# FFTAI/Wiki-GRx-Gym

Hardware: AMD Instinct MI355X
Metric: env-steps/sec GR1T1 rough-terrain @4096 envs (higher is better)
Workload: dtype f32

## Files before the change

### include/grx_ppo.h

```cpp
#ifndef GRX_PPO_H
#define GRX_PPO_H
#ifdef __cplusplus
extern "C" {
#endif

int grx_ppo_loss_partials_size(int batch);

int grx_ppo_loss(int batch, int num_actions, const float* mu, const float* std, const float* value,
                 const float* actions, const float* old_logp, const float* old_mu, const float* old_sigma,
                 const float* advantages, const float* returns, const float* target_values,
                 float clip_param, float value_loss_coef, float entropy_coef, int use_clipped_value_loss,
                 float* out, float* d_mu, float* d_std, float* d_value, float* partials, void* stream);

int grx_ppo_colsum_partials_size(int rows, int cols);
int grx_ppo_colsum(int rows, int cols, const float* x, float* out, float* partials, void* stream);

int grx_ppo_elu_backward_colsum(int rows, int cols, const float* dy, const float* y, float* dz, float* out, float* partials, void* stream);

int grx_ppo_store_transition(int N, int num_obs, int num_pri, int num_actions,
                             const float* obs, const float* pri, const float* actions, const float* mu, const float* sigma,
                             const float* values, const float* logp, const float* rewards, const unsigned char* dones,
                             const unsigned char* time_outs, float gamma,
                             float* st_obs, float* st_pri, float* st_actions, float* st_mu, float* st_sigma, float* st_values,
                             float* st_logp, float* st_rewards, unsigned char* st_dones,
                             float* cur_rew, float* cur_len, float* done_rew, float* done_len, void* stream);

#define GRX_PPO_TAIL_MAX 24
typedef struct grx_ppo_tail_tensors {
    int n, pad;
    float* param[GRX_PPO_TAIL_MAX]; const float* grad[GRX_PPO_TAIL_MAX]; float* exp_avg[GRX_PPO_TAIL_MAX]; float* exp_avg_sq[GRX_PPO_TAIL_MAX];
    float* step[GRX_PPO_TAIL_MAX];
    long long numel[GRX_PPO_TAIL_MAX];
} grx_ppo_tail_tensors;
typedef struct grx_ppo_tail_args {
    const float* loss;
    const float* bad_flag;
    const float* kl;
    float* lr;
    const float *value_loss, *surrogate_loss;
    float* sums;
    float* partials;
    int adaptive, pad;
    float desired_kl, lr_min, lr_max, max_grad_norm;
    double beta1, beta2, eps;
} grx_ppo_tail_args;
int grx_ppo_step_tail_blocks(const grx_ppo_tail_tensors* t);
int grx_ppo_step_tail(const grx_ppo_tail_tensors* t, const grx_ppo_tail_args* a, void* stream);

#define GRX_PPO_GATHER_MAX 12
int grx_ppo_gather_rows(int n_tensors, const float* const* src, float* const* dst, const int* widths, const long long* idx, int mb, void* stream);

int grx_mlp_layer(int M, int K, int N, const float* X, const float* W, const float* bias, float* Y, int elu, void* stream);

int grx_mlp_layer_bf16(int M, int K, int N, const float* X, const float* W, const float* bias, float* Y, int elu, void* stream);
int grx_mlp_input_grad_bf16(int M, int N, int K, const float* dZ, const float* W, float* dX, void* stream);
int grx_mlp_weight_grad_bf16_partials_size(int M, int N, int K);
int grx_mlp_weight_grad_bf16(int M, int N, int K, const float* dZ, const float* X, float* dW, float* partials, void* stream);

int grx_mlp_policy_head(int M, int K, int A, const float* X, const float* W, const float* bias, const float* std,
                        const float* eps, float* actions, float* logp, float* mu, float* sigma, void* stream);

int grx_obs_norm_partials_size(int rows, int cols);
int grx_obs_norm_moments(int rows, int cols, const float* x, float* partials, void* stream);
int grx_obs_norm_merge(int n_partials, int cols, int stride, const float* partials, long long* count, float* mean, float* var, float* std,
                       void* stream);
int grx_obs_norm_combine(int n_partials, int cols, const float* partials, float* out, void* stream);
int grx_obs_norm_apply(int rows, int cols, const float* x, const float* mean, const float* std, float eps, float* y, void* stream);
int grx_obs_norm_step(int rows, int cols, const float* x, float* partials, long long* count, float* mean, float* var, float* std, float eps,
                      float* y, void* stream);

int grx_obs_history_push(int N, int D, int H, const float* obs, const unsigned char* dones, int fill_all, const float* src, float* dst,
                         void* stream);

int grx_distill_loss_partials_size(int batch, int A);
int grx_distill_loss(int batch, int A, const float* student_mu, const float* teacher_mu, int huber, float* out, float* d_mu, float* partials,
                     void* stream);
int grx_distill_store(int N, int D, int A, const float* obs, const float* labels, const float* rewards, const unsigned char* dones,
                      float* st_obs, float* st_labels, unsigned char* st_dones,
                      float* cur_rew, float* cur_len, float* done_rew, float* done_len, void* stream);

int grx_lstm_cell(int M, int D, int H, const float* x, const float* h_prev, const float* c_prev, const unsigned char* reset,
                  const float* W_ih, const float* W_hh, const float* b_ih, const float* b_hh, float* h, float* c, float* acts, void* stream);
int grx_lstm_cell_preact(int M, int D, int H, const float* x, const float* h_prev, const unsigned char* reset, const float* W_ih,
                         const float* W_hh, const float* b_ih, const float* b_hh, float* G, void* stream);
int grx_lstm_cell_backward(int M, int H, const float* dh, const float* dc_in, const float* acts, const float* c_prev,
                           const unsigned char* reset, float* dG, float* dc_prev, void* stream);

#define GRX_SYM_MAX_WIDTH 2048
int grx_sym_gather_rows(int n_tensors, const float* const* src, float* const* dst, const int* widths, const int* modes,
                        const int* const* perm, const float* const* scale, const float* const* offset, const long long* idx, int mb,
                        void* stream);

int grx_rnd_reward_partials_size(int N);
int grx_rnd_reward(int N, int E, const float* pred, const float* targ, float gamma, float weight, float eps, float* ret, long long* count,
                   float* mean, float* var, float* std, float* rewards, float* intrinsic, float* raw, float* partials, void* stream);

#ifdef __cplusplus
}
#endif

#include "grx_ppo_noise.h"
#include "grx_ppo_smooth.h"
#include "grx_ppo_est.h"
#endif
```

### wiki-grx-gym_amd/rl/fused_loss.py

```python
import ctypes as C
import os

import torch

_LIB = None


def load_ppo_library():
    global _LIB
    if _LIB is None:
        path = os.environ.get("GRX_PPO_LIB") or os.path.join(os.path.dirname(os.path.dirname(os.path.abspath(__file__))), "csrc", "libgrx_ppo.so")
        if not os.path.exists(path):
            raise RuntimeError(f"{path} is missing: build it with `python -c 'import __graft_entry__ as g; g.build()'` "
                               "(there is no silent fallback for CUDA tensors; set GRX_PPO_FUSED_LOSS=0 to use the torch expression)")
        lib = C.CDLL(path)
        fp = C.c_void_p
        lib.grx_ppo_loss.restype = C.c_int
        lib.grx_ppo_loss.argtypes = [C.c_int, C.c_int] + [fp] * 10 + [C.c_float, C.c_float, C.c_float, C.c_int] + [fp] * 5 + [C.c_void_p]
        lib.grx_ppo_loss_partials_size.restype = C.c_int
        lib.grx_ppo_loss_partials_size.argtypes = [C.c_int]
        lib.grx_ppo_colsum.restype = C.c_int
        lib.grx_ppo_colsum.argtypes = [C.c_int, C.c_int, fp, fp, fp, C.c_void_p]
        lib.grx_ppo_colsum_partials_size.restype = C.c_int
        lib.grx_ppo_colsum_partials_size.argtypes = [C.c_int, C.c_int]
        lib.grx_ppo_store_transition.restype = C.c_int
        lib.grx_ppo_store_transition.argtypes = [C.c_int] * 4 + [fp] * 10 + [C.c_float] + [fp] * 13 + [C.c_void_p]
        lib.grx_ppo_elu_backward_colsum.restype = C.c_int
        lib.grx_ppo_elu_backward_colsum.argtypes = [C.c_int, C.c_int, fp, fp, fp, fp, fp, C.c_void_p]
        lib.grx_ppo_gather_rows.restype = C.c_int
        lib.grx_ppo_gather_rows.argtypes = [C.c_int, C.POINTER(C.c_void_p), C.POINTER(C.c_void_p), C.POINTER(C.c_int), fp, C.c_int, C.c_void_p]
        lib.grx_mlp_layer.restype = C.c_int
        lib.grx_mlp_layer.argtypes = [C.c_int] * 3 + [fp] * 4 + [C.c_int, C.c_void_p]
        lib.grx_mlp_layer_bf16.restype = C.c_int
        lib.grx_mlp_layer_bf16.argtypes = [C.c_int] * 3 + [fp] * 4 + [C.c_int, C.c_void_p]
        lib.grx_mlp_input_grad_bf16.restype = C.c_int
        lib.grx_mlp_input_grad_bf16.argtypes = [C.c_int] * 3 + [fp] * 3 + [C.c_void_p]
        lib.grx_mlp_weight_grad_bf16_partials_size.restype = C.c_int
        lib.grx_mlp_weight_grad_bf16_partials_size.argtypes = [C.c_int] * 3
        lib.grx_mlp_weight_grad_bf16.restype = C.c_int
        lib.grx_mlp_weight_grad_bf16.argtypes = [C.c_int] * 3 + [fp] * 4 + [C.c_void_p]
        lib.grx_mlp_policy_head.restype = C.c_int
        lib.grx_mlp_policy_head.argtypes = [C.c_int] * 3 + [fp] * 9 + [C.c_void_p]
        lib.grx_ppo_step_tail.restype = C.c_int
        lib.grx_ppo_step_tail.argtypes = [C.c_void_p, C.c_void_p, C.c_void_p]
        lib.grx_ppo_step_tail_blocks.restype = C.c_int
        lib.grx_ppo_step_tail_blocks.argtypes = [C.c_void_p]
        lib.grx_obs_norm_partials_size.restype = C.c_int
        lib.grx_obs_norm_partials_size.argtypes = [C.c_int, C.c_int]
        lib.grx_obs_norm_moments.restype = C.c_int
        lib.grx_obs_norm_moments.argtypes = [C.c_int, C.c_int, fp, fp, C.c_void_p]
        lib.grx_obs_norm_merge.restype = C.c_int
        lib.grx_obs_norm_merge.argtypes = [C.c_int, C.c_int, C.c_int] + [fp] * 5 + [C.c_void_p]
        lib.grx_obs_norm_combine.restype = C.c_int
        lib.grx_obs_norm_combine.argtypes = [C.c_int, C.c_int, fp, fp, C.c_void_p]
        lib.grx_obs_norm_apply.restype = C.c_int
        lib.grx_obs_norm_apply.argtypes = [C.c_int, C.c_int, fp, fp, fp, C.c_float, fp, C.c_void_p]
        lib.grx_obs_norm_step.restype = C.c_int
        lib.grx_obs_norm_step.argtypes = [C.c_int, C.c_int] + [fp] * 6 + [C.c_float, fp, C.c_void_p]
        lib.grx_obs_history_push.restype = C.c_int
        lib.grx_obs_history_push.argtypes = [C.c_int] * 3 + [fp, fp, C.c_int, fp, fp, C.c_void_p]
        lib.grx_distill_loss_partials_size.restype = C.c_int
        lib.grx_distill_loss_partials_size.argtypes = [C.c_int, C.c_int]
        lib.grx_distill_loss.restype = C.c_int
        lib.grx_distill_loss.argtypes = [C.c_int, C.c_int, fp, fp, C.c_int, fp, fp, fp, C.c_void_p]
        lib.grx_distill_store.restype = C.c_int
        lib.grx_distill_store.argtypes = [C.c_int] * 3 + [fp] * 11 + [C.c_void_p]
        pp = C.POINTER(C.c_void_p)
        lib.grx_sym_gather_rows.restype = C.c_int
        lib.grx_sym_gather_rows.argtypes = [C.c_int, pp, pp, C.POINTER(C.c_int), C.POINTER(C.c_int), pp, pp, pp, fp, C.c_int, C.c_void_p]
        lib.grx_rnd_reward_partials_size.restype = C.c_int
        lib.grx_rnd_reward_partials_size.argtypes = [C.c_int]
        lib.grx_rnd_reward.restype = C.c_int
        lib.grx_rnd_reward.argtypes = [C.c_int, C.c_int, fp, fp, C.c_float, C.c_float, C.c_float] + [fp] * 9 + [C.c_void_p]
        lib.grx_ppo_loss_sd_partials_size.restype = C.c_int
        lib.grx_ppo_loss_sd_partials_size.argtypes = [C.c_int]
        lib.grx_ppo_loss_sd.restype = C.c_int
        lib.grx_ppo_loss_sd.argtypes = [C.c_int, C.c_int, fp, C.c_int] + [fp] * 8 + [C.c_float, C.c_float, C.c_float, C.c_int] + [fp] * 4 + [C.c_void_p]
        lib.grx_mlp_policy_head_sd.restype = C.c_int
        lib.grx_mlp_policy_head_sd.argtypes = [C.c_int] * 3 + [fp] * 3 + [C.c_int] + [fp] * 5 + [C.c_void_p]
        lib.grx_smooth_gather_rows.restype = C.c_int
        lib.grx_smooth_gather_rows.argtypes = ([C.c_int, pp, pp, C.POINTER(C.c_int), fp, C.c_int, C.c_int, C.c_int, fp, C.c_int, C.c_int, fp,
                                                C.c_float, fp, C.c_void_p])
        lib.grx_smooth_loss_partials_size.restype = C.c_int
        lib.grx_smooth_loss_partials_size.argtypes = [C.c_int, C.c_int]
        lib.grx_smooth_loss.restype = C.c_int
        lib.grx_smooth_loss.argtypes = [C.c_int, C.c_int, fp, C.c_int, C.c_int, fp, C.c_float, C.c_float, fp, fp, fp, C.c_void_p]
        lib.grx_est_forward.restype = C.c_int
        lib.grx_est_forward.argtypes = [fp, C.c_int, C.c_int, fp, C.c_int, fp, C.POINTER(C.c_int), fp, fp, C.c_void_p]
        _LIB = lib
    return _LIB


TAIL_MAX = 24


class _TailTensors(C.Structure):
    _fields_ = [("n", C.c_int), ("pad", C.c_int), ("param", C.c_void_p * TAIL_MAX), ("grad", C.c_void_p * TAIL_MAX),
                ("exp_avg", C.c_void_p * TAIL_MAX), ("exp_avg_sq", C.c_void_p * TAIL_MAX), ("step", C.c_void_p * TAIL_MAX),
                ("numel", C.c_longlong * TAIL_MAX)]


class _TailArgs(C.Structure):
    _fields_ = [("loss", C.c_void_p), ("bad_flag", C.c_void_p), ("kl", C.c_void_p), ("lr", C.c_void_p), ("value_loss", C.c_void_p),
                ("surrogate_loss", C.c_void_p), ("sums", C.c_void_p), ("partials", C.c_void_p), ("adaptive", C.c_int), ("pad", C.c_int),
                ("desired_kl", C.c_float), ("lr_min", C.c_float), ("lr_max", C.c_float), ("max_grad_norm", C.c_float),
                ("beta1", C.c_double), ("beta2", C.c_double), ("eps", C.c_double)]


class StepTail:

    @staticmethod
    def supported(optimizer, params):
        g = optimizer.param_groups
        return (len(g) == 1 and len(params) <= TAIL_MAX and not g[0].get("amsgrad") and not g[0].get("maximize") and g[0].get("weight_decay", 0) == 0
                and all(p.is_cuda and p.dtype == torch.float32 and p.is_contiguous() for p in params))

    def __init__(self, optimizer, params, lr_t):
        self.lib = load_ppo_library()
        self.opt, self.params, self.lr_t = optimizer, list(params), lr_t
        self.t, self.a = _TailTensors(), _TailArgs()
        self.key, self.partials = None, None

    def _state(self, p):
        st = self.opt.state[p]
        if "exp_avg" not in st:
            st["step"] = torch.zeros((), dtype=torch.float32, device=p.device)
            st["exp_avg"] = torch.zeros_like(p, memory_format=torch.preserve_format)
            st["exp_avg_sq"] = torch.zeros_like(p, memory_format=torch.preserve_format)
        return st

    def __call__(self, loss, kl, value_loss, surrogate_loss, sums, adaptive, desired_kl, lr_min, lr_max, max_grad_norm, bad_flag=None):
        t, a = self.t, self.a
        sts = [self._state(p) for p in self.params]
        key = tuple(x.data_ptr() for p, st in zip(self.params, sts) for x in (p, st["exp_avg"], st["exp_avg_sq"], st["step"]))
        if key != self.key:
            t.n = len(self.params)
            for i, (p, st) in enumerate(zip(self.params, sts)):
                if not (st["step"].is_cuda and st["step"].dtype == torch.float32 and st["exp_avg"].is_contiguous() and st["exp_avg_sq"].is_contiguous()):
                    raise RuntimeError("StepTail: the optimizer state is not torch's fused / capturable layout")
                t.param[i], t.exp_avg[i], t.exp_avg_sq[i], t.step[i], t.numel[i] = p.data_ptr(), st["exp_avg"].data_ptr(), st["exp_avg_sq"].data_ptr(), st["step"].data_ptr(), p.numel()
            nb = self.lib.grx_ppo_step_tail_blocks(C.byref(t))
            if nb < 1:
                raise RuntimeError("grx_ppo_step_tail_blocks failed")
            self.partials = torch.empty(nb, device=self.params[0].device, dtype=torch.float32)
            self.key = key
        for i, p in enumerate(self.params):
            g = p.grad
            if g is None or not g.is_contiguous() or g.dtype != torch.float32:
                raise RuntimeError("StepTail: every parameter needs a contiguous fp32 .grad")
            t.grad[i] = g.data_ptr()
        g0 = self.opt.param_groups[0]
        a.loss, a.kl, a.lr = loss.data_ptr(), kl.data_ptr(), self.lr_t.data_ptr()
        a.bad_flag = bad_flag.data_ptr() if bad_flag is not None else None
        a.value_loss, a.surrogate_loss = value_loss.data_ptr(), surrogate_loss.data_ptr()
        a.sums = sums.data_ptr() if sums is not None else None
        a.partials = self.partials.data_ptr()
        a.adaptive = int(bool(adaptive))
        a.desired_kl, a.lr_min, a.lr_max, a.max_grad_norm = float(desired_kl or 0.0), float(lr_min), float(lr_max), float(max_grad_norm)
        a.beta1, a.beta2, a.eps = float(g0["betas"][0]), float(g0["betas"][1]), float(g0["eps"])
        dev = self.params[0].device
        with torch.cuda.device(dev):
            rc = self.lib.grx_ppo_step_tail(C.byref(t), C.byref(a), C.c_void_p(torch.cuda.current_stream(dev).cuda_stream))
        if rc != 0:
            raise RuntimeError(f"grx_ppo_step_tail failed ({rc})")


def _f32c(x):
    return x if (x.dtype == torch.float32 and x.is_contiguous()) else x.contiguous().float()


class FusedPPOLoss(torch.autograd.Function):

    @staticmethod
    def forward(ctx, mu, std, value, actions, old_logp, old_mu, old_sigma, advantages, returns, target_values,
                clip_param, value_loss_coef, entropy_coef, use_clipped_value_loss):
        lib = load_ppo_library()
        B, A = mu.shape
        mu_c, std_c, value_c = _f32c(mu), _f32c(std), _f32c(value).reshape(-1)
        data = [_f32c(t) for t in (actions, old_logp, old_mu, old_sigma, advantages, returns, target_values)]
        out = torch.empty(4, device=mu.device, dtype=torch.float32)
        d_mu = torch.empty_like(mu_c)
        d_std = torch.empty_like(std_c)
        d_value = torch.empty_like(value_c)
        partials = torch.empty(lib.grx_ppo_loss_partials_size(B), device=mu.device, dtype=torch.float32)
        stream = torch.cuda.current_stream(mu.device).cuda_stream
        with torch.cuda.device(mu.device):
            rc = lib.grx_ppo_loss(B, A, mu_c.data_ptr(), std_c.data_ptr(), value_c.data_ptr(), *[t.data_ptr() for t in data],
                                  float(clip_param), float(value_loss_coef), float(entropy_coef), int(bool(use_clipped_value_loss)),
                                  out.data_ptr(), d_mu.data_ptr(), d_std.data_ptr(), d_value.data_ptr(), partials.data_ptr(), C.c_void_p(stream))
        if rc != 0:
            raise RuntimeError(f"grx_ppo_loss failed ({rc}): batch {B}, num_actions {A}")
        ctx.save_for_backward(d_mu, d_std, d_value)
        ctx.value_shape = value.shape
        return out

    @staticmethod
    def backward(ctx, g):
        d_mu, d_std, d_value = ctx.saved_tensors
        gl = g[2]
        return (d_mu * gl, d_std * gl, (d_value * gl).reshape(ctx.value_shape)) + (None,) * 11


def fused_ppo_loss(mu, std, value, actions, old_logp, old_mu, old_sigma, advantages, returns, target_values,
                   clip_param, value_loss_coef, entropy_coef, use_clipped_value_loss):
    return FusedPPOLoss.apply(mu, std, value, actions, old_logp, old_mu, old_sigma, advantages, returns, target_values,
                              clip_param, value_loss_coef, entropy_coef, use_clipped_value_loss)


class FusedPPOLossSD(torch.autograd.Function):

    @staticmethod
    def forward(ctx, raw, value, actions, old_logp, old_mu, old_sigma, advantages, returns, target_values,
                log_std, clip_param, value_loss_coef, entropy_coef, use_clipped_value_loss):
        lib = load_ppo_library()
        B, A = actions.shape
        if tuple(raw.shape) != (B, 2 * A):
            raise RuntimeError(f"fused_ppo_loss_sd: raw is {tuple(raw.shape)}, expected {(B, 2 * A)} ([mean | s] of {A} actions)")
        raw_c, value_c = _f32c(raw), _f32c(value).reshape(-1)
        data = [_f32c(t) for t in (actions, old_logp, old_mu, old_sigma, advantages, returns, target_values)]
        out = torch.empty(4, device=raw.device, dtype=torch.float32)
        d_raw = torch.empty_like(raw_c)
        d_value = torch.empty_like(value_c)
        partials = torch.empty(lib.grx_ppo_loss_sd_partials_size(B), device=raw.device, dtype=torch.float32)
        stream = torch.cuda.current_stream(raw.device).cuda_stream
        with torch.cuda.device(raw.device):
            rc = lib.grx_ppo_loss_sd(B, A, raw_c.data_ptr(), int(bool(log_std)), value_c.data_ptr(), *[t.data_ptr() for t in data],
                                     float(clip_param), float(value_loss_coef), float(entropy_coef), int(bool(use_clipped_value_loss)),
                                     out.data_ptr(), d_raw.data_ptr(), d_value.data_ptr(), partials.data_ptr(), C.c_void_p(stream))
        if rc != 0:
            raise RuntimeError(f"grx_ppo_loss_sd failed ({rc}): batch {B}, num_actions {A}")
        ctx.save_for_backward(d_raw, d_value)
        ctx.value_shape = value.shape
        return out

    @staticmethod
    def backward(ctx, g):
        d_raw, d_value = ctx.saved_tensors
        gl = g[2]
        return (d_raw * gl, (d_value * gl).reshape(ctx.value_shape)) + (None,) * 12


def fused_ppo_loss_sd(raw, value, actions, old_logp, old_mu, old_sigma, advantages, returns, target_values,
                      log_std, clip_param, value_loss_coef, entropy_coef, use_clipped_value_loss):
    return FusedPPOLossSD.apply(raw, value, actions, old_logp, old_mu, old_sigma, advantages, returns, target_values,
                                log_std, clip_param, value_loss_coef, entropy_coef, use_clipped_value_loss)


def colsum(x):
    lib = load_ppo_library()
    x = _f32c(x)
    rows, cols = x.shape
    out = torch.empty(cols, device=x.device, dtype=torch.float32)
    partials = torch.empty(lib.grx_ppo_colsum_partials_size(rows, cols), device=x.device, dtype=torch.float32)
    with torch.cuda.device(x.device):
        rc = lib.grx_ppo_colsum(rows, cols, x.data_ptr(), out.data_ptr(), partials.data_ptr(),
                                C.c_void_p(torch.cuda.current_stream(x.device).cuda_stream))
    if rc != 0:
        raise RuntimeError(f"grx_ppo_colsum failed ({rc}): {rows} x {cols}")
    return out


def elu_backward_colsum(dy, y):
    lib = load_ppo_library()
    dy, y = _f32c(dy), _f32c(y)
    rows, cols = dy.shape
    dz = torch.empty_like(dy)
    out = torch.empty(cols, device=dy.device, dtype=torch.float32)
    partials = torch.empty(lib.grx_ppo_colsum_partials_size(rows, cols), device=dy.device, dtype=torch.float32)
    with torch.cuda.device(dy.device):
        rc = lib.grx_ppo_elu_backward_colsum(rows, cols, dy.data_ptr(), y.data_ptr(), dz.data_ptr(), out.data_ptr(), partials.data_ptr(),
                                             C.c_void_p(torch.cuda.current_stream(dy.device).cuda_stream))
    if rc != 0:
        raise RuntimeError(f"grx_ppo_elu_backward_colsum failed ({rc}): {rows} x {cols}")
    return dz, out


def store_transition(storage, step, obs, pri, actions, mu, sigma, values, logp, rewards, dones, time_outs, gamma, log=None):
    lib = load_ppo_library()
    N = storage.num_envs
    ptr = lambda t: t.data_ptr() if t is not None else None
    for t in (obs, pri, actions, mu, sigma, values, logp, rewards):
        if t is not None and not (t.is_cuda and t.dtype == torch.float32 and t.is_contiguous()):
            raise RuntimeError("store_transition needs contiguous float32 CUDA tensors")
    def as_u8(t):
        if t.dtype == torch.bool:
            t = t.view(torch.uint8)
        elif t.dtype != torch.uint8:
            t = (t != 0).to(torch.uint8)
        if not (t.is_cuda and t.is_contiguous() and t.numel() == N):
            raise RuntimeError("store_transition needs contiguous CUDA dones / time_outs with one entry per env")
        return t
    d8 = as_u8(dones)
    t8 = None if time_outs is None else as_u8(time_outs)
    sp = storage.pri_observations
    lg = log if log is not None else (None, None, None, None)
    with torch.cuda.device(obs.device):
        rc = lib.grx_ppo_store_transition(
            N, obs.shape[1], pri.shape[1] if (pri is not None and sp is not None) else 0, actions.shape[1],
            ptr(obs), ptr(pri) if sp is not None else None, ptr(actions), ptr(mu), ptr(sigma), ptr(values), ptr(logp), ptr(rewards), ptr(d8), ptr(t8),
            float(gamma), ptr(storage.observations[step]), ptr(sp[step]) if sp is not None else None, ptr(storage.actions[step]), ptr(storage.mu[step]),
            ptr(storage.sigma[step]), ptr(storage.values[step]), ptr(storage.actions_log_prob[step]), ptr(storage.rewards[step]), ptr(storage.dones[step]),
            ptr(lg[0]), ptr(lg[1]), ptr(lg[2]), ptr(lg[3]), C.c_void_p(torch.cuda.current_stream(obs.device).cuda_stream))
    if rc != 0:
        raise RuntimeError(f"grx_ppo_store_transition failed ({rc})")


def _linears_of(mlp):
    mods = list(mlp.model)
    lin = []
    for i, m in enumerate(mods):
        if i % 2 == 0:
            if not isinstance(m, torch.nn.Linear):
                return None
            lin.append((m.weight, m.bias))
        elif not (isinstance(m, torch.nn.ELU) and m.alpha == 1.0):
            return None
    return lin if len(mods) % 2 == 1 else None


def mlp_can_fuse(mlp, x):
    return x.is_cuda and x.dtype == torch.float32 and x.dim() == 2 and _linears_of(mlp) is not None


def _layer(lib, x, w, b, elu, stream, bf16=False):
    y = torch.empty(x.shape[0], w.shape[0], device=x.device, dtype=torch.float32)
    fn = lib.grx_mlp_layer_bf16 if bf16 else lib.grx_mlp_layer
    rc = fn(x.shape[0], x.shape[1], w.shape[0], x.data_ptr(), w.data_ptr(), b.data_ptr() if b is not None else None, y.data_ptr(), int(elu), stream)
    if rc:
        raise RuntimeError(f"{'grx_mlp_layer_bf16' if bf16 else 'grx_mlp_layer'} failed ({rc}): {tuple(x.shape)} x {tuple(w.shape)}")
    return y


def _bf16_hidden(mlp):
    return getattr(mlp, "precision", "fp32") == "bf16"


def linear_elu(x, weight, bias, bf16=False):
    lib = load_ppo_library()
    with torch.cuda.device(x.device):
        return _layer(lib, _f32c(x), _f32c(weight), bias, True, torch.cuda.current_stream(x.device).cuda_stream, bf16)


def input_grad_bf16(dz, weight):
    lib = load_ppo_library()
    dz, weight = _f32c(dz), _f32c(weight)
    (M, N), K = dz.shape, weight.shape[1]
    dx = torch.empty(M, K, device=dz.device, dtype=torch.float32)
    with torch.cuda.device(dz.device):
        rc = lib.grx_mlp_input_grad_bf16(M, N, K, dz.data_ptr(), weight.data_ptr(), dx.data_ptr(),
                                         C.c_void_p(torch.cuda.current_stream(dz.device).cuda_stream))
    if rc:
        raise RuntimeError(f"grx_mlp_input_grad_bf16 failed ({rc}): {M} x {N} x {K}")
    return dx


def weight_grad_bf16(dz, x):
    lib = load_ppo_library()
    dz, x = _f32c(dz), _f32c(x)
    (M, N), K = dz.shape, x.shape[1]
    dw = torch.empty(N, K, device=dz.device, dtype=torch.float32)
    partials = torch.empty(max(1, lib.grx_mlp_weight_grad_bf16_partials_size(M, N, K)), device=dz.device, dtype=torch.float32)
    with torch.cuda.device(dz.device):
        rc = lib.grx_mlp_weight_grad_bf16(M, N, K, dz.data_ptr(), x.data_ptr(), dw.data_ptr(), partials.data_ptr(),
                                          C.c_void_p(torch.cuda.current_stream(dz.device).cuda_stream))
    if rc:
        raise RuntimeError(f"grx_mlp_weight_grad_bf16 failed ({rc}): {M} x {N} x {K}")
    return dw


def mlp_forward(mlp, x):
    lib = load_ppo_library()
    lin = _linears_of(mlp)
    bf16 = _bf16_hidden(mlp)
    x = _f32c(x)
    stream = torch.cuda.current_stream(x.device).cuda_stream
    with torch.cuda.device(x.device):
        for i, (w, b) in enumerate(lin):
            hidden = i + 1 < len(lin)
            x = _layer(lib, x, w, b, hidden, stream, bf16 and hidden)
    return x


def policy_act(mlp, std, x, eps, state_dependent=None):
    lib = load_ppo_library()
    lin = _linears_of(mlp)
    bf16 = _bf16_hidden(mlp)
    x = _f32c(x)
    stream = torch.cuda.current_stream(x.device).cuda_stream
    with torch.cuda.device(x.device):
        for w, b in lin[:-1]:
            x = _layer(lib, x, w, b, True, stream, bf16)
        w, b = lin[-1]
        M, A = x.shape[0], w.shape[0] // (2 if state_dependent is not None else 1)
        actions, mu, sigma = (torch.empty(M, A, device=x.device, dtype=torch.float32) for _ in range(3))
        logp = torch.empty(M, device=x.device, dtype=torch.float32)
        if state_dependent is not None:
            rc = lib.grx_mlp_policy_head_sd(M, x.shape[1], A, x.data_ptr(), _f32c(w).data_ptr(), b.data_ptr() if b is not None else None,
                                            int(state_dependent == "log"), _f32c(eps).data_ptr(), actions.data_ptr(), logp.data_ptr(),
                                            mu.data_ptr(), sigma.data_ptr(), stream)
            if rc:
                raise RuntimeError(f"grx_mlp_policy_head_sd failed ({rc})")
            return actions, logp, mu, sigma
        rc = lib.grx_mlp_policy_head(M, x.shape[1], A, x.data_ptr(), w.data_ptr(), b.data_ptr() if b is not None else None,
                                     _f32c(std).data_ptr(), _f32c(eps).data_ptr(), actions.data_ptr(), logp.data_ptr(),
                                     mu.data_ptr(), sigma.data_ptr(), stream)
        if rc:
            raise RuntimeError(f"grx_mlp_policy_head failed ({rc})")
    return actions, logp, mu, sigma


class RowGather:

    def __init__(self, srcs, dsts):
        self.lib = load_ppo_library()
        n = len(srcs)
        assert n == len(dsts) and all(s.dtype == torch.float32 and s.is_contiguous() and d.is_contiguous() and d.dtype == torch.float32
                                      and s.shape[1:] == d.shape[1:] for s, d in zip(srcs, dsts))
        self.n, self.mb, self.device = n, dsts[0].shape[0], srcs[0].device
        self.src = (C.c_void_p * n)(*[s.data_ptr() for s in srcs])
        self.dst = (C.c_void_p * n)(*[d.data_ptr() for d in dsts])
        self.w = (C.c_int * n)(*[int(s[0].numel()) for s in srcs])
        self.keep = (srcs, dsts)

    def __call__(self, idx):
        assert idx.dtype == torch.int64 and idx.is_contiguous() and idx.numel() == self.mb
        with torch.cuda.device(self.device):
            rc = self.lib.grx_ppo_gather_rows(self.n, self.src, self.dst, self.w, idx.data_ptr(), self.mb,
                                              torch.cuda.current_stream(self.device).cuda_stream)
        if rc:
            raise RuntimeError(f"grx_ppo_gather_rows failed ({rc})")


class SymGather:

    def __init__(self, srcs, dsts, modes, maps):
        self.lib = load_ppo_library()
        n = len(srcs)
        assert n == len(dsts) == len(modes) == len(maps)
        rows = [d.shape[0] // (2 if m else 1) for d, m in zip(dsts, modes)]
        assert all(s.dtype == torch.float32 and s.is_contiguous() and d.is_contiguous() and d.dtype == torch.float32 and s.shape[1:] == d.shape[1:]
                   and d.shape[0] == r * (2 if m else 1) and r == rows[0] for s, d, m, r in zip(srcs, dsts, modes, rows))
        self.n, self.mb, self.device = n, rows[0], srcs[0].device
        self.src = (C.c_void_p * n)(*[s.data_ptr() for s in srcs])
        self.dst = (C.c_void_p * n)(*[d.data_ptr() for d in dsts])
        self.w = (C.c_int * n)(*[int(s[0].numel()) for s in srcs])
        self.modes = (C.c_int * n)(*[int(m) for m in modes])
        for m, mp, w in zip(modes, maps, self.w):
            assert m != 2 or (mp is not None and mp.width == w and mp.perm.dtype == torch.int32 and mp.perm.is_contiguous()
                              and mp.scale.dtype == torch.float32 and mp.scale.is_contiguous()
                              and (mp.offset is None or (mp.offset.dtype == torch.float32 and mp.offset.is_contiguous())))
        ptr = lambda t: t.data_ptr() if t is not None else None
        self.perm = (C.c_void_p * n)(*[ptr(mp.perm) if m == 2 else None for m, mp in zip(modes, maps)])
        self.scale = (C.c_void_p * n)(*[ptr(mp.scale) if m == 2 else None for m, mp in zip(modes, maps)])
        self.offset = (C.c_void_p * n)(*[ptr(mp.offset) if m == 2 else None for m, mp in zip(modes, maps)])
        self.keep = (srcs, dsts, maps)

    def __call__(self, idx=None):
        assert idx is None or (idx.dtype == torch.int64 and idx.is_contiguous() and idx.numel() == self.mb)
        with torch.cuda.device(self.device):
            rc = self.lib.grx_sym_gather_rows(self.n, self.src, self.dst, self.w, self.modes, self.perm, self.scale, self.offset,
                                              idx.data_ptr() if idx is not None else None, self.mb,
                                              torch.cuda.current_stream(self.device).cuda_stream)
        if rc:
            raise RuntimeError(f"grx_sym_gather_rows failed ({rc})")


class MirrorRows:

    def __init__(self, rows, m, device):
        self.lib = load_ppo_library()
        assert m.perm.dtype == torch.int32 and m.perm.is_contiguous() and m.scale.dtype == torch.float32 and m.scale.is_contiguous()
        self.rows, self.map, self.device = int(rows), m, device
        self.dst = torch.empty(2 * self.rows, m.width, device=device)
        self.src = (C.c_void_p * 1)(None)
        self.dstp = (C.c_void_p * 1)(self.dst.data_ptr())
        self.w, self.modes = (C.c_int * 1)(m.width), (C.c_int * 1)(2)
        self.perm, self.scale = (C.c_void_p * 1)(m.perm.data_ptr()), (C.c_void_p * 1)(m.scale.data_ptr())
        self.offset = (C.c_void_p * 1)(m.offset.data_ptr() if m.offset is not None else None)

    def __call__(self, x):
        assert x.dtype == torch.float32 and x.is_contiguous() and tuple(x.shape) == (self.rows, self.map.width) and x.device == self.dst.device
        self.src[0] = x.data_ptr()
        with torch.cuda.device(self.device):
            rc = self.lib.grx_sym_gather_rows(1, self.src, self.dstp, self.w, self.modes, self.perm, self.scale, self.offset, None, self.rows,
                                              torch.cuda.current_stream(self.device).cuda_stream)
        if rc:
            raise RuntimeError(f"grx_sym_gather_rows failed ({rc})")
        return self.dst[self.rows:]
```

### wiki-grx-gym_amd/rl/modules.py

```python
import torch
import torch.nn as nn
from torch.distributions import Normal

PRECISIONS = ("fp32", "bf16")
_ACTIVATIONS = {"elu": nn.ELU, "selu": nn.SELU, "relu": nn.ReLU, "crelu": nn.ReLU, "lrelu": nn.LeakyReLU,
                "tanh": nn.Tanh, "sigmoid": nn.Sigmoid}


def get_activation(name):
    if name not in _ACTIVATIONS:
        print("invalid activation function!")
        return None
    return _ACTIVATIONS[name]()


import os

_FUSED_ELU_FORWARD = os.environ.get("GRX_PPO_FUSED_FWD", "1") != "0"
_FUSED_ELU_BACKWARD = os.environ.get("GRX_PPO_FUSED_ELU", "1") != "0"
_TRAIN_LINEAR = os.environ.get("GRX_PPO_LINEAR", "colsum")


class _TrainLinear(torch.autograd.Function):

    @staticmethod
    def _blas(pin):
        prev = torch.backends.cuda.preferred_blas_library()
        if pin:
            torch.backends.cuda.preferred_blas_library("cublaslt")
        return prev

    @staticmethod
    def forward(ctx, x, weight, bias):
        prev = _TrainLinear._blas(weight.shape[0] == 1)
        try:
            y = torch.addmm(bias, x, weight.t())
        finally:
            torch.backends.cuda.preferred_blas_library(prev)
        ctx.save_for_backward(x, weight)
        return y

    @staticmethod
    def backward(ctx, dy):
        from .fused_loss import colsum
        x, weight = ctx.saved_tensors
        prev = _TrainLinear._blas(weight.shape[0] == 1)
        try:
            dx = dy @ weight if ctx.needs_input_grad[0] else None
            return dx, dy.t() @ x, colsum(dy)
        finally:
            torch.backends.cuda.preferred_blas_library(prev)


class _TrainLinearELU(torch.autograd.Function):

    @staticmethod
    def forward(ctx, x, weight, bias, bf16):
        ctx.bf16 = bf16
        if bf16:
            from .fused_loss import linear_elu
            y = linear_elu(x, weight, bias, bf16=True)
        elif _FUSED_ELU_FORWARD and x.is_contiguous() and weight.is_contiguous():
            from .fused_loss import linear_elu
            y = linear_elu(x, weight, bias)
        else:
            prev = _TrainLinear._blas(weight.shape[0] == 1)
            try:
                y = torch.nn.functional.elu(torch.addmm(bias, x, weight.t()))
            finally:
                torch.backends.cuda.preferred_blas_library(prev)
        ctx.save_for_backward(x, weight, y)
        return y

    @staticmethod
    def backward(ctx, dy):
        from .fused_loss import elu_backward_colsum
        x, weight, y = ctx.saved_tensors
        dz, db = elu_backward_colsum(dy, y)
        if ctx.bf16:
            from .fused_loss import input_grad_bf16, weight_grad_bf16
            dx = input_grad_bf16(dz, weight) if ctx.needs_input_grad[0] else None
            return dx, weight_grad_bf16(dz, x), db, None
        prev = _TrainLinear._blas(weight.shape[0] == 1)
        try:
            dx = dz @ weight if ctx.needs_input_grad[0] else None
            return dx, dz.t() @ x, db, None
        finally:
            torch.backends.cuda.preferred_blas_library(prev)


class MLP(nn.Module):
    def __init__(self, input_size, output_size, hidden_dims=(256, 256, 256), activation="relu", **_):
        super().__init__()
        self.input_size, self.output_size, self.hidden_dims = input_size, output_size, list(hidden_dims)
        dims = [input_size] + list(hidden_dims)
        layers = []
        for a, b in zip(dims[:-1], dims[1:]):
            layers += [nn.Linear(a, b), get_activation(activation)]
        layers.append(nn.Linear(dims[-1], output_size))
        self.model = nn.Sequential(*layers)
        self.precision = "fp32"

    def set_precision(self, precision):
        if precision not in PRECISIONS:
            raise ValueError(f"precision must be one of {PRECISIONS}, not {precision!r}")
        if precision == "bf16":
            from .fused_loss import _linears_of
            if _linears_of(self) is None:
                raise ValueError("precision='bf16' needs an MLP of Linear -> ELU(alpha=1) hidden layers")
        self.precision = precision

    @torch.jit.unused
    def _forward_bf16(self, x):
        if not (x.is_cuda and x.dtype == torch.float32):
            raise RuntimeError("an MLP set to precision='bf16' runs on a HIP device with fp32 input only (there is no CPU path)")
        if torch.is_grad_enabled():
            return self._forward_train(x, bf16=True)
        from .fused_loss import mlp_forward
        return mlp_forward(self, x.reshape(-1, x.shape[-1])).reshape(*x.shape[:-1], self.output_size)

    @torch.jit.unused
    def _forward_train(self, x, bf16=False):
        mods = list(self.model)
        i = 0
        while i < len(mods):
            m = mods[i]
            if isinstance(m, nn.Linear) and i + 1 < len(mods) and isinstance(mods[i + 1], nn.ELU) and mods[i + 1].alpha == 1.0 \
                    and (_FUSED_ELU_BACKWARD or bf16):
                x = _TrainLinearELU.apply(x, m.weight, m.bias, bf16)
                i += 2
                continue
            x = _TrainLinear.apply(x, m.weight, m.bias) if isinstance(m, nn.Linear) else m(x)
            i += 1
        return x

    def forward(self, x):
        if not torch.jit.is_scripting():
            if self.precision == "bf16":
                return self._forward_bf16(x)
            if x.is_cuda and torch.is_grad_enabled() and x.dtype == torch.float32 and _TRAIN_LINEAR == "colsum":
                return self._forward_train(x)
        return self.model(x)


NOISE_STD_TYPES = ("scalar", "log")


class MeanHead(nn.Module):

    def __init__(self, actor, num_actions: int):
        super().__init__()
        self.actor, self.num_actions = actor, int(num_actions)

    def forward(self, x):
        return torch.narrow(self.actor(x), -1, 0, self.num_actions)


class ActorCriticMLP(nn.Module):

    def __init__(self, actor_num_input, critic_num_input, actor_num_output, actor_hidden_dims=(256, 256, 256),
                 critic_hidden_dims=(256, 256, 256), activation="elu", fixed_std=False, init_noise_std=1.0,
                 set_std=True, set_noise_std=1.0, actor_output_activation=None, critic_output_activation=None, actor_output_gain=1.0,
                 noise_std_type="scalar", state_dependent_std=False, **kwargs):
        if kwargs:
            print("ActorCritic.__init__ got unexpected arguments, which will be ignored: " + str(list(kwargs)))
        if noise_std_type not in NOISE_STD_TYPES:
            raise ValueError(f"noise_std_type must be one of {NOISE_STD_TYPES}, not {noise_std_type!r}")
        state_dependent_std = bool(state_dependent_std)
        if state_dependent_std and actor_output_activation is not None:
            raise ValueError(f"state_dependent_std with actor_output_activation={actor_output_activation!r}: the output layer is [mean | s], "
                             "an activation on it is not defined")
        if state_dependent_std and fixed_std:
            raise ValueError("state_dependent_std with fixed_std: the actor emits its own sigma, there is no parameter to fix")
        super().__init__()
        self.noise_std_type, self.state_dependent_std = noise_std_type, state_dependent_std
        self.num_actor_input, self.num_actor_output = actor_num_input, actor_num_output
        self.num_critic_input, self.num_critic_output = critic_num_input, 1
        self.actor = MLP(actor_num_input, 2 * actor_num_output if state_dependent_std else actor_num_output, actor_hidden_dims, activation)
        self.critic = MLP(critic_num_input, 1, critic_hidden_dims, activation)
        A = actor_num_output
        init = torch.as_tensor(init_noise_std, dtype=torch.float32) * torch.ones(A)
        last = [m for m in self.actor.model if isinstance(m, nn.Linear)][-1]
        if actor_output_gain != 1.0:
            with torch.no_grad():
                last.weight[:A].mul_(float(actor_output_gain)); last.bias[:A].mul_(float(actor_output_gain))
        if state_dependent_std:
            with torch.no_grad():
                last.weight[A:].zero_()
                last.bias[A:].copy_(torch.log(init + 1e-7) if noise_std_type == "log" else init)
        self.fixed_std, self.init_noise_std = fixed_std, init_noise_std
        if not state_dependent_std and noise_std_type == "log":
            self.log_std = nn.Parameter(torch.log(init))
        elif not state_dependent_std:
            self.std = nn.Parameter(init.clone())
        self.register_buffer("init_std", init.clone(), persistent=False)
        self.set_std, self.set_noise_std = set_std, set_noise_std
        self.distribution = None
        Normal.set_default_validate_args = False

    is_recurrent = False

    def noise_std(self):
        if self.state_dependent_std:
            raise RuntimeError("state_dependent_std: sigma is a function of the state (the actor's second output half), there is no [A] sigma")
        if self.fixed_std:
            return self.init_std
        return torch.exp(self.log_std) if self.noise_std_type == "log" else self.std

    def split_raw(self, raw):
        A = self.num_actor_output
        s = raw[..., A:]
        return raw[..., :A], (torch.exp(s) if self.noise_std_type == "log" else s)

    def inference_actor(self):
        return MeanHead(self.actor, self.num_actor_output) if self.state_dependent_std else self.actor

    def assign_noise_std(self, std):
        if self.state_dependent_std:
            raise RuntimeError("state_dependent_std: there is no noise parameter to set")
        with torch.no_grad():
            if self.noise_std_type == "log":
                self.log_std.copy_(torch.log(std))
            else:
                self.std.copy_(std)

    def load_state_dict(self, state_dict, strict=True):
        state_dict = dict(state_dict)
        if self.state_dependent_std:
            return super().load_state_dict(state_dict, strict)
        if self.noise_std_type == "log":
            if self.fixed_std:
                with torch.no_grad():
                    self.log_std.copy_(torch.log(torch.as_tensor(self.init_noise_std, dtype=torch.float32) * torch.ones_like(self.log_std)))
                self.log_std.requires_grad = False
                state_dict["log_std"] = self.log_std.detach().clone()
            return super().load_state_dict(state_dict, strict)
        if self.set_std:
            state_dict["std"] = torch.ones_like(state_dict["std"]) * self.set_noise_std
        if self.fixed_std:
            with torch.no_grad():
                self.std.copy_(torch.as_tensor(self.init_noise_std, dtype=torch.float32) * torch.ones_like(self.std))
            self.std.requires_grad = False
            state_dict["std"] = self.std.detach().clone()
        return super().load_state_dict(state_dict, strict)

    def set_precision(self, precision):
        self.actor.set_precision(precision)
        self.critic.set_precision(precision)

    def reset(self, dones=None):
        pass

    def forward(self, *a, **k):
        raise NotImplementedError

    @property
    def action_mean(self):
        return self.distribution.mean

    @property
    def action_std(self):
        return self.distribution.stddev

    @property
    def entropy(self):
        return self.distribution.entropy().sum(dim=-1)

    def update_distribution(self, observations):
        if self.state_dependent_std:
            mean, std = self.split_raw(self.actor(observations))
            self.distribution = Normal(mean, std)
            return
        mean = self.actor(observations)
        std = self.noise_std().to(mean.device)
        self.distribution = Normal(mean, mean * 0.0 + std)

    def act(self, observations, **_):
        self.update_distribution(observations)
        return self.distribution.sample()

    def get_actions_log_prob(self, actions):
        return self.distribution.log_prob(actions).sum(dim=-1)

    def act_inference(self, observations):
        if self.state_dependent_std:
            return self.actor(observations)[..., :self.num_actor_output]
        return self.actor(observations)

    def evaluate(self, critic_observations=None, **_):
        return self.critic(critic_observations)
```

Measured before the change: 96.98 million.

## Fuse narrow output head forward and backward with last ELU layer in training MLP

Adds custom HIP kernels for the narrow final Linear head (up to 32 outputs). The forward pass is a tiled small-N GEMV-like kernel. The backward kernel computes the input gradient through the ELU, dW, db and the ELU bias colsum in one pass, followed by a deterministic double-precision reduction of per-slab partials. The last hidden Linear+ELU and the head are wrapped in one autograd function, replacing several BLAS calls and colsum kernels for skinny matrices. The risk is that the custom kernels are slower than tuned BLAS for these shapes, and the partials buffer is allocated on every backward call.

```diff
diff --git a/include/grx_ppo.h b/include/grx_ppo.h
--- a/include/grx_ppo.h
+++ b/include/grx_ppo.h
@@ -102,4 +102,5 @@
 #include "grx_ppo_noise.h"
 #include "grx_ppo_smooth.h"
 #include "grx_ppo_est.h"
+#include "grx_ppo_head.h"
 #endif
diff --git a/include/grx_ppo_head.h b/include/grx_ppo_head.h
--- /dev/null
+++ b/include/grx_ppo_head.h
@@ -0,0 +1,18 @@
+#ifndef GRX_PPO_HEAD_H
+#define GRX_PPO_HEAD_H
+
+#define GRX_HEAD_MAX_A 32
+
+#ifdef __cplusplus
+extern "C" {
+#endif
+
+int grx_head_forward(int M, int K, int A, const float* X, const float* W, const float* bias, float* out, void* stream);
+int grx_head_backward_partials_size(int M, int K, int A);
+int grx_head_backward(int M, int K, int A, const float* d_out, const float* X, const float* W, int elu, float* dZ, float* dW, float* db,
+                      float* dbz, float* partials, void* stream);
+
+#ifdef __cplusplus
+}
+#endif
+#endif
diff --git a/wiki-grx-gym_amd/csrc/grx_ppo_head.hip b/wiki-grx-gym_amd/csrc/grx_ppo_head.hip
--- /dev/null
+++ b/wiki-grx-gym_amd/csrc/grx_ppo_head.hip
@@ -0,0 +1,219 @@
+#include <hip/hip_runtime.h>
+#include <stdint.h>
+#include "../../include/grx_ppo_head.h"
+
+namespace {
+
+constexpr int HF_ROWS = 32, HF_KC = 128, HF_LD = HF_KC + 1;
+
+template <int NA, bool VEC>
+__global__ __launch_bounds__(256) void head_forward_kernel(int M, int K, int A, const float* __restrict__ X, const float* __restrict__ W,
+                                                           const float* __restrict__ bias, float* __restrict__ out) {
+    __shared__ float s_x[HF_ROWS * HF_LD];
+    __shared__ float s_w[GRX_HEAD_MAX_A * HF_KC];
+    const int tid = threadIdx.x, r = tid & 31, g = tid >> 5;
+    const int m0 = blockIdx.x * HF_ROWS;
+    float acc[NA];
+    int wrow[NA];
+#pragma unroll
+    for (int j = 0; j < NA; ++j) { acc[j] = 0.f; wrow[j] = min(g + 8 * j, A - 1) * HF_KC; }
+    for (int k0 = 0; k0 < K; k0 += HF_KC) {
+        const int kc = min(HF_KC, K - k0);
+        if (VEC) {
+            for (int i = tid; i < HF_ROWS * (HF_KC / 4); i += 256) {
+                const int rr = i / (HF_KC / 4), c = (i % (HF_KC / 4)) * 4, m = m0 + rr;
+                float4 v = make_float4(0.f, 0.f, 0.f, 0.f);
+                if (m < M && c < kc) v = *reinterpret_cast<const float4*>(X + (size_t)m * K + k0 + c);
+                float* d = s_x + rr * HF_LD + c;
+                d[0] = v.x; d[1] = v.y; d[2] = v.z; d[3] = v.w;
+            }
+        } else {
+            for (int i = tid; i < HF_ROWS * HF_KC; i += 256) {
+                const int rr = i / HF_KC, c = i % HF_KC, m = m0 + rr;
+                s_x[rr * HF_LD + c] = (m < M && c < kc) ? X[(size_t)m * K + k0 + c] : 0.f;
+            }
+        }
+        for (int i = tid; i < A * HF_KC; i += 256) {
+            const int a = i / HF_KC, c = i % HF_KC;
+            s_w[i] = c < kc ? W[(size_t)a * K + k0 + c] : 0.f;
+        }
+        __syncthreads();
+        const float* xr = s_x + r * HF_LD;
+        for (int k = 0; k < kc; ++k) {
+            const float x = xr[k];
+#pragma unroll
+            for (int j = 0; j < NA; ++j) acc[j] = fmaf(x, s_w[wrow[j] + k], acc[j]);
+        }
+        __syncthreads();
+    }
+    const int m = m0 + r;
+    if (m < M) {
+#pragma unroll
+        for (int j = 0; j < NA; ++j) {
+            const int a = g + 8 * j;
+            if (a < A) out[(size_t)m * A + a] = bias ? acc[j] + bias[a] : acc[j];
+        }
+    }
+}
+
+template <int NA>
+void launch_forward(bool vec, int M, int K, int A, const float* X, const float* W, const float* bias, float* out, hipStream_t st) {
+    const dim3 grid((M + HF_ROWS - 1) / HF_ROWS);
+    if (vec) hipLaunchKernelGGL((head_forward_kernel<NA, true>), grid, dim3(256), 0, st, M, K, A, X, W, bias, out);
+    else hipLaunchKernelGGL((head_forward_kernel<NA, false>), grid, dim3(256), 0, st, M, K, A, X, W, bias, out);
+}
+
+constexpr int HB_MAX_ROWS = 256, HB_MIN_ROWS = 32, HB_BLOCKS = 512, HB_UNROLL = 8;
+
+int hb_slab_rows(int M, int K) {
+    const long long nct = ((long long)K + 63) / 64;
+    const long long want = nct >= HB_BLOCKS ? 1 : (HB_BLOCKS + nct - 1) / nct;
+    long long rows = (M + want - 1) / want;
+    rows = (rows + 3) & ~3LL;
+    if (rows < HB_MIN_ROWS) rows = HB_MIN_ROWS;
+    if (rows > HB_MAX_ROWS) rows = HB_MAX_ROWS;
+    return (int)rows;
+}
+
+template <int AB>
+__global__ __launch_bounds__(256) void head_backward_kernel(int M, int K, int A, int slab_rows, int elu, const float* __restrict__ d_out,
+                                                            const float* __restrict__ X, const float* __restrict__ W, float* __restrict__ dZ,
+                                                            float* __restrict__ partials) {
+    __shared__ __attribute__((aligned(16))) float s_d[HB_MAX_ROWS * AB];
+    __shared__ float s_red[3][AB + 1][64];
+    __shared__ float s_db[4][AB];
+    const int tid = threadIdx.x, lane = tid & 63, wv = tid >> 6;
+    const long long kk = (long long)blockIdx.x * 64 + lane;
+    const bool valid = kk < K, first = blockIdx.x == 0;
+    const int k = valid ? (int)kk : 0;
+    const int r0 = blockIdx.y * slab_rows, nrows = min(slab_rows, M - r0);
+    for (int i = tid; i < nrows * AB; i += 256) {
+        const int rr = i / AB, a = i % AB;
+        s_d[i] = a < A ? d_out[(size_t)(r0 + rr) * A + a] : 0.f;
+    }
+    float w[AB], dw[AB], dbs[AB];
+#pragma unroll
+    for (int a = 0; a < AB; ++a) { w[a] = (valid && a < A) ? W[(size_t)a * K + k] : 0.f; dw[a] = 0.f; dbs[a] = 0.f; }
+    float dbz = 0.f;
+    __syncthreads();
+    for (int rb = wv; rb < nrows; rb += 4 * HB_UNROLL) {
+        float xs[HB_UNROLL];
+#pragma unroll
+        for (int u = 0; u < HB_UNROLL; ++u) {
+            const int rr = rb + 4 * u;
+            xs[u] = (valid && rr < nrows) ? X[(size_t)(r0 + rr) * K + k] : 0.f;
+        }
+#pragma unroll
+        for (int u = 0; u < HB_UNROLL; ++u) {
+            const int rr = rb + 4 * u;
+            if (rr < nrows) {
+                float dv[AB];
+#pragma unroll
+                for (int a = 0; a < AB; a += 4) {
+                    const float4 t = *reinterpret_cast<const float4*>(s_d + rr * AB + a);
+                    dv[a] = t.x; dv[a + 1] = t.y; dv[a + 2] = t.z; dv[a + 3] = t.w;
+                }
+                float dot = 0.f;
+#pragma unroll
+                for (int a = 0; a < AB; ++a) dot = fmaf(dv[a], w[a], dot);
+                const float x = xs[u];
+                const float dz = dot * (elu ? (x > 0.f ? 1.0f : x + 1.0f) : 1.0f);
+                if (valid) dZ[(size_t)(r0 + rr) * K + k] = dz;
+                dbz += dz;
+#pragma unroll
+                for (int a = 0; a < AB; ++a) dw[a] = fmaf(dv[a], x, dw[a]);
+                if (first) {
+#pragma unroll
+                    for (int a = 0; a < AB; ++a) dbs[a] += dv[a];
+                }
+            }
+        }
+    }
+    if (wv > 0) {
+#pragma unroll
+        for (int a = 0; a < AB; ++a) s_red[wv - 1][a][lane] = dw[a];
+        s_red[wv - 1][AB][lane] = dbz;
+    }
+    if (first && lane == 0) {
+#pragma unroll
+        for (int a = 0; a < AB; ++a) s_db[wv][a] = dbs[a];
+    }
+    __syncthreads();
+    if (wv != 0) return;
+    const size_t AK = (size_t)A * K;
+    float* p = partials + (size_t)blockIdx.y * (AK + A + K);
+    if (valid) {
+#pragma unroll
+        for (int a = 0; a < AB; ++a)
+            if (a < A) p[(size_t)a * K + k] = ((dw[a] + s_red[0][a][lane]) + s_red[1][a][lane]) + s_red[2][a][lane];
+        p[AK + A + k] = ((dbz + s_red[0][AB][lane]) + s_red[1][AB][lane]) + s_red[2][AB][lane];
+    }
+    if (first && lane < A) p[AK + lane] = ((s_db[0][lane] + s_db[1][lane]) + s_db[2][lane]) + s_db[3][lane];
+}
+
+constexpr int HB_FJ = 16, HB_FG = 16;
+__global__ __launch_bounds__(256) void head_backward_final(int nslab, int P, int AK, int A, int n_out, const float* __restrict__ partials,
+                                                           float* __restrict__ dW, float* __restrict__ db, float* __restrict__ dbz) {
+    __shared__ double s_f[HB_FG][HB_FJ];
+    const int jl = threadIdx.x % HB_FJ, g = threadIdx.x / HB_FJ;
+    const int j = blockIdx.x * HB_FJ + jl;
+    const int s0 = (int)((long long)g * nslab / HB_FG), s1 = (int)((long long)(g + 1) * nslab / HB_FG);
+    double acc = 0.0;
+    if (j < n_out) {
+#pragma unroll 8
+        for (int s = s0; s < s1; ++s) acc += (double)partials[(size_t)s * P + j];
+    }
+    s_f[g][jl] = acc;
+    __syncthreads();
+    if (g != 0 || j >= n_out) return;
+    double t = s_f[0][jl];
+#pragma unroll
+    for (int q = 1; q < HB_FG; ++q) t += s_f[q][jl];
+    const float v = (float)t;
+    if (j < AK) dW[j] = v;
+    else if (j < AK + A) db[j - AK] = v;
+    else dbz[j - AK - A] = v;
+}
+
+bool hb_shape_ok(int M, int K, int A) {
+    if (M < 1 || K < 1 || A < 1 || A > GRX_HEAD_MAX_A) return false;
+    const long long P = (long long)A * K + A + K;
+    const long long nslab = ((long long)M + hb_slab_rows(M, K) - 1) / hb_slab_rows(M, K);
+    return P < (1LL << 31) && nslab <= 65535 && nslab * P < (1LL << 31);
+}
+
+}
+
+extern "C" int grx_head_forward(int M, int K, int A, const float* X, const float* W, const float* bias, float* out, void* stream) {
+    if (M < 1 || K < 1 || A < 1 || A > GRX_HEAD_MAX_A || !X || !W || !out) return -1;
+    const bool vec = K % 4 == 0 && (uintptr_t)X % 16 == 0;
+    const hipStream_t st = (hipStream_t)stream;
+    switch ((A + 7) / 8) {
+        case 1: launch_forward<1>(vec, M, K, A, X, W, bias, out, st); break;
+        case 2: launch_forward<2>(vec, M, K, A, X, W, bias, out, st); break;
+        case 3: launch_forward<3>(vec, M, K, A, X, W, bias, out, st); break;
+        default: launch_forward<4>(vec, M, K, A, X, W, bias, out, st); break;
+    }
+    return hipGetLastError() == hipSuccess ? 0 : -2;
+}
+
+extern "C" int grx_head_backward_partials_size(int M, int K, int A) {
+    if (!hb_shape_ok(M, K, A)) return 0;
+    const int rows = hb_slab_rows(M, K);
+    return (int)((((long long)M + rows - 1) / rows) * ((long long)A * K + A + K));
+}
+
+extern "C" int grx_head_backward(int M, int K, int A, const float* d_out, const float* X, const float* W, int elu, float* dZ, float* dW,
+                                 float* db, float* dbz, float* partials, void* stream) {
+    if (!hb_shape_ok(M, K, A) || !d_out || !X || !W || !dZ || !dW || !db || !partials || (elu && !dbz)) return -1;
+    const hipStream_t st = (hipStream_t)stream;
+    const int rows = hb_slab_rows(M, K), nslab = (M + rows - 1) / rows;
+    const dim3 grid((K + 63) / 64, nslab);
+    if (A <= 8) hipLaunchKernelGGL(head_backward_kernel<8>, grid, dim3(256), 0, st, M, K, A, rows, elu ? 1 : 0, d_out, X, W, dZ, partials);
+    else if (A <= 16) hipLaunchKernelGGL(head_backward_kernel<16>, grid, dim3(256), 0, st, M, K, A, rows, elu ? 1 : 0, d_out, X, W, dZ, partials);
+    else hipLaunchKernelGGL(head_backward_kernel<32>, grid, dim3(256), 0, st, M, K, A, rows, elu ? 1 : 0, d_out, X, W, dZ, partials);
+    if (hipGetLastError() != hipSuccess) return -2;
+    const int AK = A * K, P = AK + A + K, n_out = elu ? P : AK + A;
+    hipLaunchKernelGGL(head_backward_final, dim3((n_out + HB_FJ - 1) / HB_FJ), dim3(256), 0, st, nslab, P, AK, A, n_out, partials, dW, db, dbz);
+    return hipGetLastError() == hipSuccess ? 0 : -2;
+}
diff --git a/wiki-grx-gym_amd/rl/fused_loss.py b/wiki-grx-gym_amd/rl/fused_loss.py
--- a/wiki-grx-gym_amd/rl/fused_loss.py
+++ b/wiki-grx-gym_amd/rl/fused_loss.py
@@ -87,6 +87,12 @@
         lib.grx_smooth_loss.argtypes = [C.c_int, C.c_int, fp, C.c_int, C.c_int, fp, C.c_float, C.c_float, fp, fp, fp, C.c_void_p]
         lib.grx_est_forward.restype = C.c_int
         lib.grx_est_forward.argtypes = [fp, C.c_int, C.c_int, fp, C.c_int, fp, C.POINTER(C.c_int), fp, fp, C.c_void_p]
+        lib.grx_head_forward.restype = C.c_int
+        lib.grx_head_forward.argtypes = [C.c_int] * 3 + [fp] * 4 + [C.c_void_p]
+        lib.grx_head_backward_partials_size.restype = C.c_int
+        lib.grx_head_backward_partials_size.argtypes = [C.c_int] * 3
+        lib.grx_head_backward.restype = C.c_int
+        lib.grx_head_backward.argtypes = [C.c_int] * 3 + [fp] * 3 + [C.c_int] + [fp] * 5 + [C.c_void_p]
         _LIB = lib
     return _LIB
 
@@ -275,6 +281,54 @@
     return dz, out
 
 
+HEAD_MAX_OUT = 32
+
+
+def head_forward_torch(x, weight, bias):
+    y = x @ weight.t()
+    return y if bias is None else y + bias
+
+
+def head_backward_torch(d_out, x, weight, elu):
+    dz = d_out @ weight
+    if elu:
+        dz = dz * torch.where(x > 0, torch.ones_like(x), x + 1.0)
+    return dz, d_out.t() @ x, d_out.sum(0), (dz.sum(0) if elu else None)
+
+
+def head_forward(x, weight, bias):
+    lib = load_ppo_library()
+    x, weight = _f32c(x), _f32c(weight)
+    bias = None if bias is None else _f32c(bias)
+    (M, K), A = x.shape, weight.shape[0]
+    out = torch.empty(M, A, device=x.device, dtype=torch.float32)
+    with torch.cuda.device(x.device):
+        rc = lib.grx_head_forward(M, K, A, x.data_ptr(), weight.data_ptr(), bias.data_ptr() if bias is not None else None, out.data_ptr(),
+                                  C.c_void_p(torch.cuda.current_stream(x.device).cuda_stream))
+    if rc != 0:
+        raise RuntimeError(f"grx_head_forward failed ({rc}): {M} x {K} x {A}")
+    return out
+
+
+def head_backward(d_out, x, weight, elu):
+    lib = load_ppo_library()
+    d_out, x, weight = _f32c(d_out), _f32c(x), _f32c(weight)
+    (M, K), A = x.shape, weight.shape[0]
+    dev = x.device
+    dz = torch.empty_like(x)
+    dw = torch.empty(A, K, device=dev, dtype=torch.float32)
+    db = torch.empty(A, device=dev, dtype=torch.float32)
+    dbz = torch.empty(K, device=dev, dtype=torch.float32) if elu else None
+    partials = torch.empty(max(1, lib.grx_head_backward_partials_size(M, K, A)), device=dev, dtype=torch.float32)
+    with torch.cuda.device(dev):
+        rc = lib.grx_head_backward(M, K, A, d_out.data_ptr(), x.data_ptr(), weight.data_ptr(), int(bool(elu)), dz.data_ptr(), dw.data_ptr(),
+                                   db.data_ptr(), dbz.data_ptr() if elu else None, partials.data_ptr(),
+                                   C.c_void_p(torch.cuda.current_stream(dev).cuda_stream))
+    if rc != 0:
+        raise RuntimeError(f"grx_head_backward failed ({rc}): {M} x {K} x {A}")
+    return dz, dw, db, dbz
+
+
 def store_transition(storage, step, obs, pri, actions, mu, sigma, values, logp, rewards, dones, time_outs, gamma, log=None):
     lib = load_ppo_library()
     N = storage.num_envs
diff --git a/wiki-grx-gym_amd/rl/modules.py b/wiki-grx-gym_amd/rl/modules.py
--- a/wiki-grx-gym_amd/rl/modules.py
+++ b/wiki-grx-gym_amd/rl/modules.py
@@ -19,6 +19,7 @@
 _FUSED_ELU_FORWARD = os.environ.get("GRX_PPO_FUSED_FWD", "1") != "0"
 _FUSED_ELU_BACKWARD = os.environ.get("GRX_PPO_FUSED_ELU", "1") != "0"
 _TRAIN_LINEAR = os.environ.get("GRX_PPO_LINEAR", "colsum")
+_FUSED_HEAD = os.environ.get("GRX_PPO_FUSED_HEAD", "1") != "0"
 
 
 class _TrainLinear(torch.autograd.Function):
@@ -89,6 +90,33 @@
             torch.backends.cuda.preferred_blas_library(prev)
 
 
+class _TrainHiddenHead(torch.autograd.Function):
+
+    @staticmethod
+    def forward(ctx, x, w1, b1, w2, b2, bf16):
+        from .fused_loss import head_forward, linear_elu
+        ctx.bf16 = bf16
+        h = linear_elu(x, w1, b1, bf16=bf16)
+        ctx.save_for_backward(x, w1, h, w2)
+        return head_forward(h, w2, b2)
+
+    @staticmethod
+    def backward(ctx, dy):
+        from .fused_loss import head_backward
+        x, w1, h, w2 = ctx.saved_tensors
+        dz, dw2, db2, db1 = head_backward(dy, h, w2, elu=True)
+        if ctx.bf16:
+            from .fused_loss import input_grad_bf16, weight_grad_bf16
+            dx = input_grad_bf16(dz, w1) if ctx.needs_input_grad[0] else None
+            return dx, weight_grad_bf16(dz, x), db1, dw2, db2, None
+        prev = _TrainLinear._blas(w1.shape[0] == 1)
+        try:
+            dx = dz @ w1 if ctx.needs_input_grad[0] else None
+            return dx, dz.t() @ x, db1, dw2, db2, None
+        finally:
+            torch.backends.cuda.preferred_blas_library(prev)
+
+
 class MLP(nn.Module):
     def __init__(self, input_size, output_size, hidden_dims=(256, 256, 256), activation="relu", **_):
         super().__init__()
@@ -119,12 +147,28 @@
         from .fused_loss import mlp_forward
         return mlp_forward(self, x.reshape(-1, x.shape[-1])).reshape(*x.shape[:-1], self.output_size)
 
+    @staticmethod
+    def _ends_in_narrow_head(mods, x, bf16):
+        from .fused_loss import HEAD_MAX_OUT
+        hid, act, head = mods[-3:]
+        if not (_FUSED_HEAD and (bf16 or (_FUSED_ELU_BACKWARD and _FUSED_ELU_FORWARD))):
+            return False
+        if not (isinstance(hid, nn.Linear) and isinstance(act, nn.ELU) and act.alpha == 1.0 and isinstance(head, nn.Linear)):
+            return False
+        if head.out_features > HEAD_MAX_OUT or hid.bias is None or head.bias is None:
+            return False
+        tensors = (x, hid.weight, hid.bias, head.weight, head.bias)
+        return x.dim() == 2 and all(t.is_cuda and t.dtype == torch.float32 and t.is_contiguous() for t in tensors)
+
     @torch.jit.unused
     def _forward_train(self, x, bf16=False):
         mods = list(self.model)
         i = 0
         while i < len(mods):
             m = mods[i]
+            if i + 3 == len(mods) and self._ends_in_narrow_head(mods, x, bf16):
+                head = mods[i + 2]
+                return _TrainHiddenHead.apply(x, m.weight, m.bias, head.weight, head.bias, bf16)
             if isinstance(m, nn.Linear) and i + 1 < len(mods) and isinstance(mods[i + 1], nn.ELU) and mods[i + 1].alpha == 1.0 \
                     and (_FUSED_ELU_BACKWARD or bf16):
                 x = _TrainLinearELU.apply(x, m.weight, m.bias, bf16)
```

Measured after the change: 96.88 million. No clear change (-0.1%).
